# MarvinLvn/CPC2

Measured on AMD Instinct MI355X. Metric: audio-seconds/sec CPC training (1.28 s @16 kHz, 128 neg), higher is better.
Workload: dtype f32

## Files before the change

cpc2_amd/_lib.py:

```python
import ctypes
import os
import time

import torch

_HERE = os.path.dirname(os.path.abspath(__file__))
LIB_PATH = os.environ.get("CPC2_HIP_LIB") or os.path.join(_HERE, "libcpc2_hip.so")

c_float_p = ctypes.c_void_p
c_ptr = ctypes.c_void_p
c_int = ctypes.c_int
c_long = ctypes.c_long
c_size_t = ctypes.c_size_t
c_float = ctypes.c_float

SIGNATURES = {
    "cpc_version": (c_int, []),
    "cpc_last_error": (ctypes.c_char_p, []),
    "cpc_async_error_check": (c_int, [c_ptr]),
    "cpc_prof_enable": (c_int, [c_int]),
    "cpc_gemm_set_mode": (c_int, [c_int]),
    "cpc_prof_read": (c_int, [ctypes.c_char_p, ctypes.POINTER(ctypes.c_double), ctypes.POINTER(c_long)]),
    "cpc_gemm_nt": (c_int, [c_ptr, c_long, c_ptr, c_long, c_ptr, c_long, c_ptr, c_int, c_int, c_int, c_ptr]),
    "cpc_gemm_tn_scratch_bytes": (c_size_t, [c_int, c_int, c_long]),
# ... 42 lines not shown
    "cpc_negidx_sample_host": (c_int, [c_ptr, c_int, c_int, c_int, c_int, c_int, c_ptr, c_ptr, c_ptr]),
    "cpc_negidx_sample_host_async": (c_int, [c_ptr, c_int, c_int, c_int, c_int, c_int, c_ptr]),
    "cpc_negidx_wait": (c_int, [c_ptr]),
    "cpc_mt_draw_host": (c_int, [c_ptr, c_ptr, c_size_t]),
    "cpc_mt_draw_host_async": (c_int, [c_ptr, c_ptr, c_size_t]),
    "cpc_mt_draw_device_async": (c_int, [c_ptr, c_ptr, c_ptr, c_size_t, c_int, c_ptr]),
    "cpc_mt_draw_expand_device_async": (c_int, [c_ptr, c_ptr, c_ptr, c_ptr, c_int, c_int, c_int, c_int, c_int, c_ptr]),
    "cpc_mt_redraw_expand_device_async": (c_int, [c_ptr, c_ptr, c_int, c_int, c_size_t, c_ptr, c_ptr, c_ptr, c_int, c_int, c_int, c_int, c_int, c_ptr]),
    "cpc_negidx_wait_on": (c_int, [c_ptr, c_ptr]),
    "cpc_negidx_stream": (c_int, [c_ptr, c_ptr]),
    "cpc_stream_create_apart": (c_int, [c_ptr, c_int, c_ptr]),
    "cpc_streams_overlap": (c_int, [c_ptr, c_ptr]),
    "cpc_stream_apart_failures": (c_long, []),
    "cpc_stream_spin": (c_int, [c_ptr, c_long]),
    "cpc_side_stream": (c_int, [c_ptr, c_ptr]),
    "cpc_negidx_expand": (c_int, [c_ptr, c_ptr, c_int, c_int, c_int, c_int, c_ptr]),
    "cpc_infonce_saved_bytes": (c_size_t, [c_int] * 6),
    "cpc_infonce_scratch_bytes": (c_size_t, [c_int] * 6),
    "cpc_infonce_logits_offset": (c_size_t, [c_int] * 6),
    "cpc_infonce_perm_offset": (c_size_t, [c_int] * 6),
    "cpc_infonce_forward": (c_int, [c_ptr] * 9 + [c_int] * 7 + [c_ptr]),
    "cpc_infonce_backward": (c_int, [c_ptr] * 11 + [c_int] * 8 + [c_ptr]),
    "cpc_infonce_join": (c_int, [c_ptr]),
    "cpc_infonce_forward_pred": (c_int, [c_ptr] * 8 + [c_int] * 5 + [c_ptr]),
    "cpc_infonce_backward_pred": (c_int, [c_ptr] * 9 + [c_int] * 5 + [c_ptr]),
    "cpc_flac_info": (c_int, [ctypes.c_char_p, ctypes.POINTER(c_int), ctypes.POINTER(c_int), ctypes.POINTER(c_int),
                              ctypes.POINTER(c_long)]),
    "cpc_flac_decode_f32": (c_int, [ctypes.c_char_p, c_ptr, c_long, ctypes.POINTER(c_int)]),
    "cpc_window_gather": (c_int, [c_ptr, c_long, c_ptr, c_ptr, c_int, c_int, c_ptr]),
    "cpc_adam_step": (c_int, [c_ptr, c_ptr, c_ptr, c_ptr, c_long, c_int, c_float, c_float, c_float, c_float, c_float, c_ptr]),
    "cpc_sgd_step": (c_int, [c_ptr, c_ptr, c_ptr, c_long, c_int, c_float, c_float, c_float, c_ptr]),
    "cpc_abx_dtw_scratch_bytes": (c_size_t, [c_int, c_int, c_int]),
    "cpc_abx_dtw": (c_int, [c_ptr, c_int, c_ptr, c_ptr, c_int, c_ptr, c_ptr, c_ptr, c_int, c_int, c_int, c_int, c_ptr, c_ptr,
                            c_ptr, c_size_t, c_ptr]),
    "cpc_abx_counts": (c_int, [c_ptr, c_int, c_ptr, c_ptr, c_ptr, c_int, c_ptr, c_ptr, c_ptr]),
    "cpc_abx_dtw_units_scratch_bytes": (c_size_t, [c_int, c_int, c_int]),
    "cpc_abx_dtw_units": (c_int, [c_ptr, c_ptr, c_ptr, c_int, c_ptr, c_ptr, c_ptr, c_int, c_int, c_int, c_float, c_float, c_ptr,
                                  c_ptr, c_ptr, c_size_t, c_ptr]),
    "cpc_kmeans_scratch_bytes": (c_size_t, [c_long, c_int, c_int]),
    "cpc_kmeans_assign": (c_int, [c_ptr, c_long, c_int, c_ptr, c_int, c_ptr, c_ptr, c_ptr]),
    "cpc_kmeans_distances": (c_int, [c_ptr, c_long, c_int, c_ptr, c_int, c_ptr, c_ptr]),
    "cpc_kmeans_accumulate": (c_int, [c_ptr, c_long, c_int, c_ptr, c_int, c_ptr, c_ptr, c_ptr, c_size_t, c_ptr]),
    "cpc_probe_xent": (c_int, [c_ptr, c_ptr, c_long, c_int, c_int, c_ptr, c_ptr, c_ptr, c_ptr, c_ptr]),
    "cpc_probe_xent_backward_scratch_bytes": (c_size_t, [c_int]),
    "cpc_probe_head_backward": (c_int, [c_ptr, c_long, c_int, c_ptr, c_ptr, c_ptr, c_size_t, c_ptr]),
    "cpc_probe_ctc_scratch_bytes": (c_size_t, [c_int, c_int, c_int]),
# ... 117 lines not shown
```

cpc2_amd/csrc/infonce.hip:

```cpp
#include "common.h"
#include <hip/hip_ext.h>
#include "coop.h"
#include "ldsdma.h"
#include "rowcfg.h"

#include <algorithm>
#include <atomic>
#include <cstdlib>
#include <map>
#include <mutex>

namespace cpc {

typedef float f32x4 __attribute__((ext_vector_type(4)));
typedef float f32x16 __attribute__((ext_vector_type(16)));

constexpr int NCE_ROWS = 16;
constexpr int NCE_POS = 16;

struct NceArgs {
    const float *Pk[16];
    float *dPk[16];
    long p_stride;
    int p_rows;
    int p_packed;
    const float *z;
    const int32_t *ext;
    const unsigned short *perm;
    const float *weights;
    float *logits;
    float *lse;
    float *lossp;
    float *hit;
    int b, T, W, K, Nneg;
    int lw;
    const float *dloss;
    float *vbuf;
    float *ds_buf;
    float inv_count;
};

__global__ __launch_bounds__(64) void nce_block_sort_kernel(const int32_t *ext, int32_t *sorted, unsigned short *perm, int Nneg,
                                                            int rows_per_block, int nblk, int nrows, int *err)
{
    const long base = (long)blockIdx.x * Nneg;
    const int lane = threadIdx.x;
    int pos = 0;
    bool bad = false;
    for (int blk = 0; blk < nblk; ++blk)
        for (int c = 0; c < Nneg; c += 64) {
            const int j = c + lane;
            int row = j < Nneg ? ext[base + j] : -1;
            if (j < Nneg && (unsigned)row >= (unsigned)nrows) { bad = true; row = 0; }
            const bool mine = j < Nneg && min(row / rows_per_block, nblk - 1) == blk;
            const unsigned long long m = __ballot(mine);
            if (mine) {
                const int at = pos + __popcll(m & ((1ull << lane) - 1ull));
                sorted[base + at] = row;
                perm[base + at] = (unsigned short)j;
            }
            pos += __popcll(m);
// ... 467 lines not shown
#pragma unroll
        for (int kp = 0; kp < NCE_ROWS / 2; ++kp) av[kp] = dS[(2 * kp + h) * a.lw + ct * 32 + r32];
        int voff[16];
#pragma unroll
        for (int e = 0; e < 16; ++e) {
            const int ci = ct * 32 + (e & 3) + 8 * (e >> 2) + 4 * h;
            voff[e] = rowidx[ci] >= 0 ? (ci < NCE_POS ? ci : ci - NCE_POS + a.K) * H : -1;
        }
#pragma unroll
        for (int dt = 0; dt < DT32; ++dt) {
            f32x16 acc;
#pragma unroll
            for (int e = 0; e < 16; ++e) acc[e] = 0.f;
#pragma unroll
            for (int kp = 0; kp < NCE_ROWS / 2; ++kp) acc = __builtin_amdgcn_mfma_f32_32x32x2f32(av[kp], bvals[dt][kp], acc, 0, 0, 0);
#pragma unroll
            for (int e = 0; e < 16; ++e)
                if (voff[e] >= 0) vb[voff[e] + dt * 32] = acc[e];
        }
    }
}

constexpr int NCE_SROW = 68;
template <int H, int NKK> __global__ __launch_bounds__(H / 2) void infonce_bwd_fused_kernel(NceArgs a)
{
    constexpr int NW = H / 128;
    extern __shared__ __attribute__((aligned(16))) float smem[];
    float *dS = smem;
    int *rowidx = reinterpret_cast<int *>(dS + NCE_ROWS * a.lw);
    float *stage0 = reinterpret_cast<float *>(rowidx + a.lw);
    const int wave = threadIdx.x >> 6, lane = threadIdx.x & 63, r = lane & 15, q = lane >> 4;
    float *stage = stage0 + wave * 16 * NCE_SROW;

    const int bb = blockIdx.x / a.p_rows, t = blockIdx.x - bb * a.p_rows;
    if (t >= a.W) {
        for (int k = 0; k < a.K; ++k) {
            float *row = a.dPk[k] + ((long)bb * a.p_rows + t) * a.p_stride;
            for (int i = threadIdx.x; i < H / 4; i += 64 * NW) reinterpret_cast<float4 *>(row)[i] = make_float4(0.f, 0.f, 0.f, 0.f);
        }
        return;
    }
    const long bt = (long)bb * a.W + t;
    const int ncand = NCE_POS + a.Nneg;
    const int npad = a.lw - 4;
    const float inv_h = 1.f / H;
    const float wgt = (a.weights != nullptr ? a.weights[bt] : 1.f) * a.inv_count;

// ... 25 lines not shown
            const int neg = a.ext[bt * a.Nneg + j];
            const int pos = (g < a.K && t + 1 + g < a.T) ? bb * a.T + t + 1 + g : -1;
            rowidx[g] = g < NCE_POS ? pos : (g < ncand ? neg : -1);
        }
#pragma unroll
        for (int i = 0; i < NT; ++i)
            if ((int)threadIdx.x + 64 * NW * i < n) stage0[threadIdx.x + 64 * NW * i] = tmp[i];
    }
    __syncthreads();
#pragma unroll
    for (int kk = 0; kk < KW; ++kk) {
        const int k = wave + NW * kk, kc = min(k, a.K - 1);
#pragma unroll
        for (int i = 0; i < GI; ++i) {
            const int g = lane + 64 * i;
            const float e = expf(stage0[kc * lrow + gi[i]] - lsek[kk]);
            float v = g >= NCE_POS ? (g < ncand ? coef[kk] * e : 0.f) : (g == k ? coef[kk] * (e - 1.f) : 0.f);
            if (k >= a.K) v = 0.f;
            if (g < a.lw) dS[k * a.lw + g] = v;
        }
    }
    __syncthreads();

    const int d0 = 128 * wave;
    const long prow_off = ((long)bb * a.p_rows + t) * a.p_stride + d0;
    float pa[8][NKK];
#pragma unroll
    for (int kk = 0; kk < NKK; ++kk) {
        const int k = 4 * kk + q;
        const float *pk = a.Pk[min(k, a.K - 1)] + prow_off + r;
#pragma unroll
        for (int tile = 0; tile < 8; ++tile) {
            const float v = pk[16 * tile];
            pa[tile][kk] = k < a.K ? v : 0.f;
        }
    }
    float *vb = a.vbuf + (bt * (long)ncand + q) * H + d0 + 4 * r;
#define NCE_ROWS_GROUP(C0)                                                                                                     \
    {                                                                                                                          \
        const int c0_ = (C0);                                                                                                  \
        float bv[NKK];                                                                                                         \
        _Pragma("unroll") for (int kk = 0; kk < NKK; ++kk) bv[kk] = dS[(4 * kk + q) * a.lw + c0_ + r];                        \
        _Pragma("unroll") for (int half = 0; half < 2; ++half) {                                                               \
            f32x4 acc[4];                                                                                                      \
            _Pragma("unroll") for (int tl = 0; tl < 4; ++tl) acc[tl] = (f32x4){0.f, 0.f, 0.f, 0.f};                            \
            _Pragma("unroll") for (int kk = 0; kk < NKK; ++kk)                                                                 \
                _Pragma("unroll") for (int tl = 0; tl < 4; ++tl)                                                               \
                    acc[tl] = __builtin_amdgcn_mfma_f32_16x16x4f32(pa[4 * half + tl][kk], bv[kk], acc[tl], 0, 0, 0);           \
            _Pragma("unroll") for (int tl = 0; tl < 4; ++tl)                                                                   \
                *reinterpret_cast<f32x4 *>(stage + r * NCE_SROW + 16 * tl + 4 * q) = acc[tl];                                  \
            __builtin_amdgcn_fence(__ATOMIC_RELEASE, "wavefront");                                                             \
            __builtin_amdgcn_wave_barrier();                                                                                   \
            float4 v[4];                                                                                                       \
            _Pragma("unroll") for (int j = 0; j < 4; ++j)                                                                      \
                v[j] = *reinterpret_cast<const float4 *>(stage + (4 * j + q) * NCE_SROW + 4 * r);                              \
            _Pragma("unroll") for (int j = 0; j < 4; ++j)                                                                      \
                __builtin_nontemporal_store(__builtin_bit_cast(f32x4, v[j]),                                                   \
// ... 16 lines not shown
                const int g = 4 * (s0 + u) + q;
                const int row = rowidx[g];
                bv4[buf][u] = dS[r * a.lw + g];
                const float *src = a.z + (long)(row >= 0 ? row : 0) * H + d0 + 4 * r;
                av[buf][u][0] = *reinterpret_cast<const float4 *>(src);
                av[buf][u][1] = *reinterpret_cast<const float4 *>(src + 64);
            }
        };
        auto multiply = [&](int buf) {
#pragma unroll
            for (int u = 0; u < 4; ++u)
#pragma unroll
                for (int T4 = 0; T4 < 2; ++T4) {
                    dp[T4][0] = __builtin_amdgcn_mfma_f32_16x16x4f32(av[buf][u][T4].x, bv4[buf][u], dp[T4][0], 0, 0, 0);
                    dp[T4][1] = __builtin_amdgcn_mfma_f32_16x16x4f32(av[buf][u][T4].y, bv4[buf][u], dp[T4][1], 0, 0, 0);
                    dp[T4][2] = __builtin_amdgcn_mfma_f32_16x16x4f32(av[buf][u][T4].z, bv4[buf][u], dp[T4][2], 0, 0, 0);
                    dp[T4][3] = __builtin_amdgcn_mfma_f32_16x16x4f32(av[buf][u][T4].w, bv4[buf][u], dp[T4][3], 0, 0, 0);
                }
        };
        const int nb = npad / 16;
        request(0, 0);
        for (int ib = 0; ib < nb; ib += 2) {
            request(1, 4 * (ib + 1));
            NCE_ROWS_GROUP(16 * ib)
            multiply(0);
            if (ib + 2 < nb) request(0, 4 * (ib + 2));
            if (16 * (ib + 1) < ncand) NCE_ROWS_GROUP(16 * (ib + 1))
            multiply(1);
        }
        if (r < a.K) {
            float *dprow = a.dPk[r] + ((long)bb * a.p_rows + t) * a.p_stride + d0;
#pragma unroll
            for (int T4 = 0; T4 < 2; ++T4)
#pragma unroll
                for (int reg = 0; reg < 4; ++reg)
                    *reinterpret_cast<float4 *>(dprow + 64 * T4 + 16 * q + 4 * reg) =
                        make_float4(dp[T4][0][reg], dp[T4][1][reg], dp[T4][2][reg], dp[T4][3][reg]);
        }
    }
#undef NCE_ROWS_GROUP
}

__global__ void nce_hist_kernel(const int32_t *ext, long n, int *counts)
{
    for (long o = (long)blockIdx.x * blockDim.x + threadIdx.x; o < n; o += (long)gridDim.x * blockDim.x)
        atomicAdd(counts + ext[o], 1);
}

__global__ __launch_bounds__(1024) void nce_scan_kernel(const int *counts, int rows, int *offsets)
{
// ... 85 lines not shown
        for (int i = 0; i < 8; ++i)
#pragma unroll
            for (int c = 0; c < PER; ++c)
                v[i][c] = lane + 64 * c < C4 ? nt_load4(v4 + (long)src[i] * C4 + lane + 64 * c) : make_float4(0.f, 0.f, 0.f, 0.f);
#pragma unroll
        for (int i = 0; i < 8; ++i)
#pragma unroll
            for (int c = 0; c < PER; ++c) { acc[c].x += v[i][c].x; acc[c].y += v[i][c].y; acc[c].z += v[i][c].z; acc[c].w += v[i][c].w; }
    }
    for (; e > beg; --e) {
        const int o = entries[e - 1];
        add_row((long)(o / Nneg) * vrows + pos_rows + o % Nneg);
    }
    for (int k = 0; k < K; ++k) {
        const int t = tp - 1 - k;
        if (t >= 0 && t < W) add_row(((long)bb * W + t) * vrows + k);
    }
#pragma unroll
    for (int c = 0; c < PER; ++c)
        if (lane + 64 * c < C4) reinterpret_cast<float4 *>(dz)[(long)r * C4 + lane + 64 * c] = acc[c];
    }
}

__global__ void negidx_expand_kernel(const uint32_t *raw, int32_t *ext, int b, int T, int W, int Nneg)
{
    const long n = (long)b * Nneg * W;
    for (long o = (long)blockIdx.x * blockDim.x + threadIdx.x; o < n; o += (long)gridDim.x * blockDim.x) {
        const int nn = (int)(o % Nneg);
        const long bt = o / Nneg;
        const int t = (int)(bt % W), bb = (int)(bt / W);
        const long i = ((long)bb * Nneg + nn) * W + t;
        const uint32_t bi = raw[i] % (uint32_t)b;
        uint32_t seq = raw[n + i] % (uint32_t)(T - 1) + 1u + (uint32_t)t;
        if (seq >= (uint32_t)T) seq -= (uint32_t)T;
        ext[o] = (int32_t)(seq + bi * (uint32_t)T);
    }
}

struct NceLayout {
    int b, T, K, W, Har, Henc, Nneg, lw;
    int Pr;
    float *P, *logits, *lse;
    int32_t *ext_sorted;
    unsigned short *perm;
    int nblk, rows_per_block;
    size_t saved_bytes;
    float *lossp, *hit, *dP, *wt, *tn, *tn_late;
    float *vbuf;
    float *ds_buf;
    int *counts, *offsets, *entries;
    size_t tn_bytes, scratch_bytes;
    size_t lds_fwd, lds_bwd, lds_bwd_fused;
};

static bool nce_supported(int H) { return H == 32 || H == 64 || H == 128 || H == 256 || H == 512; }

static int nce_layout(NceLayout &l, int b, int T, int K, int Har, int Henc, int Nneg, void *saved, void *scratch)
{
    CPC_REQUIRE(nce_supported(Henc), "infonce: encoder dim %d not supported (32, 64, 128, 256, 512)", Henc);
    CPC_REQUIRE(b > 0 && K >= 1 && K <= 16 && T > K && Nneg >= 1 && Har >= 1,
                "infonce: bad shape b=%d T=%d K=%d (1..16) dim_ar=%d n_neg=%d", b, T, K, Har, Nneg);
    l.b = b; l.T = T; l.K = K; l.W = T - K; l.Har = Har; l.Henc = Henc; l.Nneg = Nneg; l.Pr = T;
    l.lw = (int)cdiv(NCE_POS + Nneg, 32) * 32 + 4;
    Carver sv(saved);
    l.P = sv.take<float>((size_t)b * T * K * Henc);
    l.logits = sv.take<float>((size_t)b * l.W * K * (Nneg + 1));
    l.lse = sv.take<float>((size_t)b * l.W * K);
    l.ext_sorted = sv.take<int32_t>((size_t)b * l.W * Nneg);
    l.perm = sv.take<unsigned short>((size_t)b * l.W * Nneg + 1024);
    const size_t zbytes = sizeof(float) * (size_t)b * T * Henc;
    l.nblk = (int)std::min<size_t>(16, std::max<size_t>(1, (zbytes + (1u << 21) - 1) >> 21));
    l.rows_per_block = (int)cdiv((long)b * T, l.nblk);
    l.saved_bytes = sv.used();
    Carver sc(scratch);
    l.lossp = sc.take<float>((size_t)b * l.W * K);
    l.hit = sc.take<float>((size_t)b * l.W * K);
    l.dP = sc.take<float>((size_t)b * T * K * Henc);
    l.wt = sc.take<float>((size_t)K * Henc * Har);
    l.tn_bytes = std::max(gemm_tn_scratch_bytes(K * Henc, Har, (long)b * T), gemm_nt_scratch_bytes((long)b * T, Har, K * Henc));
    l.tn = sc.take<float>(l.tn_bytes / sizeof(float));
    l.tn_late = sc.take<float>(l.tn_bytes / sizeof(float));
    l.counts = sc.take<int>((size_t)b * T);
    l.offsets = sc.take<int>((size_t)b * T + 1);
    l.entries = sc.take<int>((size_t)b * l.W * Nneg);
    l.vbuf = sc.take<float>((size_t)b * l.W * (NCE_POS + Nneg) * Henc);
    l.ds_buf = sc.take<float>((size_t)b * l.W * (NCE_ROWS + 1) * l.lw);
    l.scratch_bytes = sc.used();
    l.lds_fwd = align_up(sizeof(int) * (size_t)Nneg + sizeof(unsigned short) * (size_t)Nneg, 16);
    l.lds_bwd = sizeof(float) * (size_t)NCE_ROWS * l.lw + sizeof(int) * (size_t)l.lw;
    CPC_REQUIRE(l.lds_bwd <= 64 * 1024, "infonce: n_neg=%d needs %zu B of LDS (> 64 KiB)", Nneg, l.lds_bwd);
    l.lds_bwd_fused = l.lds_bwd + sizeof(float) * (size_t)(Henc / 128) * 16 * NCE_SROW;
    return CPC_OK;
}

template <typename Kern> static int allow_lds(Kern kern, size_t bytes)
{
    if (bytes > 64 * 1024)
        CPC_CHECK_HIP(hipFuncSetAttribute(reinterpret_cast<const void *>(kern), hipFuncAttributeMaxDynamicSharedMemorySize, (int)bytes));
    return CPC_OK;
}

#define NCE_DISPATCH(H, ...)                                    \
    switch (H) {                                                \
    case 32: { constexpr int HH = 32; __VA_ARGS__; } break;    \
    case 64: { constexpr int HH = 64; __VA_ARGS__; } break;    \
    case 128: { constexpr int HH = 128; __VA_ARGS__; } break;  \
    case 256: { constexpr int HH = 256; __VA_ARGS__; } break;  \
    case 512: { constexpr int HH = 512; __VA_ARGS__; } break;  \
    default: break;                                             \
// ... 41 lines not shown
                if (status == CPC_OK && e0 != nullptr) hipExtLaunchKernelGGL(infonce_fwd_dma_kernel<512>, dim3(grid), dim3(64), lds, st, e0, e1, 0, a, n_bt);
                else if (status == CPC_OK) hipLaunchKernelGGL(infonce_fwd_dma_kernel<512>, dim3(grid), dim3(64), lds, st, a, n_bt);
            }
        } else {
            NCE_DISPATCH(l.Henc, {
                status = allow_lds(infonce_fwd_kernel<HH>, l.lds_fwd);
                if (status == CPC_OK) hipLaunchKernelGGL(infonce_fwd_kernel<HH>, dim3((unsigned)(l.b * l.W)), dim3(64), l.lds_fwd, st, a);
            });
        }
        if (status != CPC_OK) prof.cancel();
    }
    CPC_TRY(status);
    CPC_CHECK_LAUNCH("infonce_fwd_kernel");
    hipLaunchKernelGGL(infonce_reduce_kernel, dim3(2 * l.K), dim3(256), 0, st, l.lossp, l.hit, (long)l.b * l.W, l.K, a.inv_count, losses, acc);
    CPC_CHECK_LAUNCH("infonce_reduce_kernel");
    return CPC_OK;
}

struct NceSide {
    hipStream_t stream = nullptr;
    hipEvent_t fork = nullptr, join = nullptr;
    hipEvent_t mid = nullptr, late = nullptr;
    std::atomic<bool> pending{false};
    bool marked = false, started = false, late_fused = false;
    NceLayout l;
    float *dz = nullptr, *dwpred = nullptr;
    const float *c = nullptr;
};

static int nce_side(NceSide **out, hipStream_t caller)
{
    static std::mutex mu;
    static std::map<int, NceSide> sides;
    int dev = 0;
    CPC_CHECK_HIP(hipGetDevice(&dev));
    std::lock_guard<std::mutex> lk(mu);
    NceSide &sd = sides[dev];
    if (sd.stream == nullptr) {
        CPC_TRY(side_stream_get(caller, &sd.stream));
        CPC_CHECK_HIP(hipEventCreateWithFlags(&sd.fork, hipEventDisableTiming));
        CPC_CHECK_HIP(hipEventCreateWithFlags(&sd.join, hipEventDisableTiming));
        CPC_CHECK_HIP(hipEventCreateWithFlags(&sd.mid, hipEventDisableTiming));
        CPC_CHECK_HIP(hipEventCreateWithFlags(&sd.late, hipEventDisableTiming));
    }
    *out = &sd;
    return CPC_OK;
}

static int nce_launch_gather(const NceLayout &l, float *dz, bool fused, hipStream_t st)
{
    const int rows = l.b * l.T;
    const unsigned wgs = (unsigned)cdiv(rows, 4);
    NCE_DISPATCH(l.Henc, hipLaunchKernelGGL(infonce_dz_gather_kernel<HH>, dim3(wgs), dim3(256), 0, st, l.vbuf,
                                             l.offsets, l.entries, dz, l.b, l.T, l.W, l.K, l.Nneg, fused ? NCE_POS : l.K));
    CPC_CHECK_LAUNCH("infonce_dz_gather_kernel");
    return CPC_OK;
}

static int nce_launch_bwd(NceArgs &a, const NceLayout &l, float *dz, hipStream_t st, NceSide **late = nullptr)
{
    const long n = (long)l.b * l.W * l.Nneg;
    const int rows = l.b * l.T;
    a.vbuf = l.vbuf;
    a.ds_buf = l.ds_buf;
    ProfScope prof(PROF_NCE_BWD, st);
    NceSide *side = nullptr;
    CPC_TRY(nce_side(&side, st));
    CPC_CHECK_HIP(hipEventRecord(side->fork, st));
    CPC_CHECK_HIP(hipStreamWaitEvent(side->stream, side->fork, 0));
    const unsigned blocks = (unsigned)std::min<long>(cdiv(n, 256), 4096);
    CPC_CHECK_HIP(hipMemsetAsync(l.counts, 0, sizeof(int) * (size_t)rows, side->stream));
    hipLaunchKernelGGL(nce_hist_kernel, dim3(blocks), dim3(256), 0, side->stream, a.ext, n, l.counts);
    hipLaunchKernelGGL(nce_scan_kernel, dim3(1), dim3(1024), 0, side->stream, l.counts, rows, l.offsets);
    CPC_CHECK_HIP(hipMemsetAsync(l.counts, 0, sizeof(int) * (size_t)rows, side->stream));
    hipLaunchKernelGGL(nce_fill_kernel, dim3(blocks), dim3(256), 0, side->stream, a.ext, n, l.offsets, l.counts, l.entries);
    hipLaunchKernelGGL(nce_sort_kernel, dim3((unsigned)cdiv(rows, 4)), dim3(256), 0, side->stream, l.offsets, l.entries, rows);
    CPC_CHECK_LAUNCH("infonce reference lists");
    CPC_CHECK_HIP(hipEventRecord(side->join, side->stream));
    int status = CPC_OK;
    const bool fused = (l.Henc == 256 || l.Henc == 512) && a.perm != nullptr && l.lw <= 320 &&
                       l.Nneg % 16 == 0 && (size_t)l.K * (l.Nneg + 1) <= (size_t)(l.Henc / 128) * 16 * NCE_SROW;
    if (fused) {
        const unsigned grid = (unsigned)(l.b * a.p_rows);
#define NCE_FUSED(HH, NKK)                                                                                                  \
    {                                                                                                                       \
        status = allow_lds(infonce_bwd_fused_kernel<HH, NKK>, l.lds_bwd_fused);                                             \
        if (status == CPC_OK) hipLaunchKernelGGL((infonce_bwd_fused_kernel<HH, NKK>), dim3(grid), dim3(HH / 2), l.lds_bwd_fused, st, a); \
    }
        const int nkk = (l.K + 3) / 4;
        if (l.Henc == 256) {
            if (nkk == 1) NCE_FUSED(256, 1) else if (nkk == 2) NCE_FUSED(256, 2) else if (nkk == 3) NCE_FUSED(256, 3) else NCE_FUSED(256, 4)
        } else {
            if (nkk == 1) NCE_FUSED(512, 1) else if (nkk == 2) NCE_FUSED(512, 2) else if (nkk == 3) NCE_FUSED(512, 3) else NCE_FUSED(512, 4)
        }
#undef NCE_FUSED
    } else {
        NCE_DISPATCH(l.Henc, {
            status = allow_lds(infonce_bwd_kernel<HH>, l.lds_bwd);
            if (status == CPC_OK) hipLaunchKernelGGL(infonce_bwd_kernel<HH>, dim3((unsigned)(l.b * a.p_rows)), dim3(64), l.lds_bwd, st, a);
        });
    }
    CPC_TRY(status);
    CPC_CHECK_LAUNCH("infonce_bwd_kernel");
    if (!fused) {
        NCE_DISPATCH(l.Henc, hipLaunchKernelGGL(infonce_dz_store_kernel<HH>, dim3((unsigned)(l.b * l.W)), dim3(64), l.lds_bwd, st, a));
        CPC_CHECK_LAUNCH("infonce_dz_store_kernel");
    }
    if (late != nullptr) {
        *late = side;
        side->late_fused = fused;
        return CPC_OK;
    }
    CPC_CHECK_HIP(hipStreamWaitEvent(st, side->join, 0));
    CPC_TRY(nce_launch_gather(l, dz, fused, st));
    return CPC_OK;
}

static int infonce_forward(const float *c, const float *z, const float *wpred, const int32_t *ext, const float *weights,
                           float *losses, float *acc, void *saved, void *scratch, int b, int T, int K, int Har, int Henc,
                           int Nneg, int c_frames, hipStream_t st)
{
    NceLayout l;
    CPC_TRY(nce_layout(l, b, T, K, Har, Henc, Nneg, saved, scratch));
    CPC_REQUIRE(c_frames == T || c_frames == l.W, "infonce: the context holds %d frames per window (expected %d or %d)", c_frames, T, l.W);
    l.Pr = c_frames;
    RowMap none{};
    CPC_TRY(gemm_nt(c, Har, wpred, Har, l.P, (long)K * Henc, nullptr, (long)b * l.Pr, K * Henc, Har, none, st));
    CPC_TRY(nce_sort_negatives(l, ext, st));
    NceArgs a{};
    nce_common(a, l, z, ext, weights);
    for (int k = 0; k < K; ++k) a.Pk[k] = l.P + (size_t)k * Henc;
    a.p_stride = (long)K * Henc; a.p_rows = l.Pr;
    a.p_packed = (size_t)b * T * K * Henc * sizeof(float) < (1ull << 32) ? 1 : 0;
    return nce_launch_fwd(a, l, losses, acc, st);
}

static int infonce_backward(const float *c, const float *z, const float *wpred, const int32_t *ext, const float *weights,
                            const float *dlosses, void *saved, void *scratch, float *dc, float *dz, float *dwpred, int b, int T,
                            int K, int Har, int Henc, int Nneg, int c_frames, bool defer, hipStream_t st)
{
    NceLayout l;
    CPC_TRY(nce_layout(l, b, T, K, Har, Henc, Nneg, saved, scratch));
    CPC_REQUIRE(c_frames == T || c_frames == l.W, "infonce: the context holds %d frames per window (expected %d or %d)", c_frames, T, l.W);
    l.Pr = c_frames;
    NceArgs a{};
    nce_common(a, l, z, ext, weights);
    for (int k = 0; k < K; ++k) { a.Pk[k] = l.P + (size_t)k * Henc; a.dPk[k] = l.dP + (size_t)k * Henc; }
    a.p_stride = (long)K * Henc; a.p_rows = l.Pr;
    a.dloss = dlosses;
    NceSide *late = nullptr;
    CPC_TRY(nce_launch_bwd(a, l, dz, st, defer ? &late : nullptr));
    CPC_TRY(transpose2d(wpred, l.wt, K * Henc, Har, st));
    RowMap none{};
    none.splitk_scratch = l.tn; none.splitk_bytes = l.tn_bytes;
    CPC_TRY(gemm_nt(l.dP, (long)K * Henc, l.wt, (long)K * Henc, dc, Har, nullptr, (long)b * l.Pr, Har, K * Henc, none, st));
    if (late != nullptr) {
        late->l = l; late->dz = dz; late->dwpred = dwpred; late->c = c;
        late->started = false; late->marked = false;
        late->pending.store(true);
    } else {
        CPC_TRY(gemm_tn(l.dP, (long)K * Henc, c, Har, dwpred, Har, K * Henc, Har, (long)b * l.Pr, l.tn, l.tn_bytes, 0, 0, st));
    }
    return CPC_OK;
}

int infonce_deferred_mark(hipStream_t st)
{
    NceSide *side = nullptr;
    CPC_TRY(nce_side(&side, st));
    if (!side->pending.load() || side->started || side->marked) return CPC_OK;
    CPC_CHECK_HIP(hipEventRecord(side->mid, st));
    side->marked = true;
    return CPC_OK;
}

int infonce_deferred_start(hipStream_t st)
{
    NceSide *side = nullptr;
    CPC_TRY(nce_side(&side, st));
    if (!side->pending.load() || side->started) return CPC_OK;
    const NceLayout &l = side->l;
    CPC_TRY(infonce_deferred_mark(st));
    CPC_CHECK_HIP(hipStreamWaitEvent(side->stream, side->mid, 0));
    CPC_TRY(nce_launch_gather(l, side->dz, side->late_fused, side->stream));
    CPC_TRY(gemm_tn(l.dP, (long)l.K * l.Henc, side->c, l.Har, side->dwpred, l.Har, l.K * l.Henc, l.Har, (long)l.b * l.Pr, l.tn_late, l.tn_bytes, 0,
                    0, side->stream));
    CPC_CHECK_HIP(hipEventRecord(side->late, side->stream));
    side->started = true;
    return CPC_OK;
}

static int infonce_join(hipStream_t st)
{
    NceSide *side = nullptr;
    CPC_TRY(nce_side(&side, st));
    if (side->pending.load()) {
        CPC_TRY(infonce_deferred_start(st));
        {
            ProfScope held(PROF_SIDE_WAIT, st);
            CPC_CHECK_HIP(hipStreamWaitEvent(st, side->late, 0));
        }
        side->pending.store(false);
    }
    return CPC_OK;
}

static int infonce_forward_pred(const float *const *pred, const float *z, const int32_t *ext, const float *weights, float *losses,
                                float *acc, void *saved, void *scratch, int b, int T, int K, int Henc, int Nneg, hipStream_t st)
{
    NceLayout l;
    CPC_TRY(nce_layout(l, b, T, K, Henc, Henc, Nneg, saved, scratch));
    CPC_TRY(nce_sort_negatives(l, ext, st));
    NceArgs a{};
    nce_common(a, l, z, ext, weights);
    for (int k = 0; k < K; ++k) a.Pk[k] = pred[k];
    a.p_stride = Henc; a.p_rows = l.W;
    return nce_launch_fwd(a, l, losses, acc, st);
}

static int infonce_backward_pred(const float *const *pred, const float *z, const int32_t *ext, const float *weights,
                                 const float *dlosses, void *saved, void *scratch, float *const *dpred, float *dz, int b, int T, int K,
                                 int Henc, int Nneg, hipStream_t st)
{
    NceLayout l;
    CPC_TRY(nce_layout(l, b, T, K, Henc, Henc, Nneg, saved, scratch));
    NceArgs a{};
    nce_common(a, l, z, ext, weights);
    for (int k = 0; k < K; ++k) { a.Pk[k] = pred[k]; a.dPk[k] = dpred[k]; }
    a.p_stride = Henc; a.p_rows = l.W;
    a.dloss = dlosses;
    return nce_launch_bwd(a, l, dz, st);
}

}

extern "C" int cpc_negidx_expand(const uint32_t *raw, int32_t *ext_idx, int batch, int seq_len, int window, int n_neg,
                                 cpc_stream_t stream)
{
    CPC_REQUIRE(raw != nullptr && ext_idx != nullptr && batch >= 1 && seq_len >= 2 && window >= 1 && window <= seq_len && n_neg >= 1 &&
                    (long long)batch * seq_len <= 2147483647LL,
                "cpc_negidx_expand: bad arguments (batch=%d seq_len=%d window=%d n_neg=%d)", batch, seq_len, window, n_neg);
    const long n = (long)batch * n_neg * window;
    hipLaunchKernelGGL(cpc::negidx_expand_kernel, dim3((unsigned)std::min<long>(cpc::cdiv(n, 256), 2048)), dim3(256), 0,
                       static_cast<hipStream_t>(stream), raw, ext_idx, batch, seq_len, window, n_neg);
    CPC_CHECK_LAUNCH("negidx_expand_kernel");
    return CPC_OK;
}

extern "C" size_t cpc_infonce_saved_bytes(int b, int t, int k, int dim_ar, int dim_enc, int n_neg)
{
    cpc::NceLayout l;
    if (cpc::nce_layout(l, b, t, k, dim_ar, dim_enc, n_neg, nullptr, nullptr) != CPC_OK) return 0;
    return l.saved_bytes;
}

extern "C" size_t cpc_infonce_logits_offset(int b, int t, int k, int dim_ar, int dim_enc, int n_neg)
{
    cpc::NceLayout l;
    char *const base = reinterpret_cast<char *>(4096);
    if (cpc::nce_layout(l, b, t, k, dim_ar, dim_enc, n_neg, base, nullptr) != CPC_OK) return (size_t)-1;
    return (size_t)(reinterpret_cast<char *>(l.logits) - base);
}

extern "C" size_t cpc_infonce_perm_offset(int b, int t, int k, int dim_ar, int dim_enc, int n_neg)
{
    cpc::NceLayout l;
    char *const base = reinterpret_cast<char *>(4096);
    if (cpc::nce_layout(l, b, t, k, dim_ar, dim_enc, n_neg, base, nullptr) != CPC_OK) return (size_t)-1;
    return (size_t)(reinterpret_cast<char *>(l.perm) - base);
}

extern "C" size_t cpc_infonce_scratch_bytes(int b, int t, int k, int dim_ar, int dim_enc, int n_neg)
{
    cpc::NceLayout l;
    if (cpc::nce_layout(l, b, t, k, dim_ar, dim_enc, n_neg, nullptr, nullptr) != CPC_OK) return 0;
    return l.scratch_bytes;
}

extern "C" int cpc_infonce_forward(const float *c, const float *z, const float *wpred, const int32_t *ext_idx, const float *weights,
                                   float *losses, float *acc, void *saved, void *scratch, int b, int t, int c_frames, int k, int dim_ar,
                                   int dim_enc, int n_neg, cpc_stream_t stream)
{
    return cpc::infonce_forward(c, z, wpred, ext_idx, weights, losses, acc, saved, scratch, b, t, k, dim_ar, dim_enc, n_neg, c_frames,
                                static_cast<hipStream_t>(stream));
}

extern "C" int cpc_infonce_backward(const float *c, const float *z, const float *wpred, const int32_t *ext_idx, const float *weights,
                                    const float *dlosses, void *saved, void *scratch, float *dc, float *dz, float *dwpred, int b,
                                    int t, int c_frames, int k, int dim_ar, int dim_enc, int n_neg, int deferred, cpc_stream_t stream)
{
    return cpc::infonce_backward(c, z, wpred, ext_idx, weights, dlosses, saved, scratch, dc, dz, dwpred, b, t, k, dim_ar, dim_enc,
                                 n_neg, c_frames, deferred != 0, static_cast<hipStream_t>(stream));
}

// ... 18 lines not shown
```

include/cpc2_hip.h:

```cpp
#ifndef CPC2_HIP_H
#define CPC2_HIP_H

#include <stddef.h>
#include <stdint.h>

#ifdef __cplusplus
extern "C" {
#endif

typedef void *cpc_stream_t;

enum cpc_status {
    CPC_OK = 0,
    CPC_ERR_INVALID = -1,
    CPC_ERR_HIP = -2,
    CPC_ERR_WORKSPACE = -3
};

int cpc_version(void);
const char *cpc_last_error(void);

int cpc_async_error_check(cpc_stream_t stream);

int cpc_stream_create_apart(const cpc_stream_t *avoid, int n_avoid, cpc_stream_t *out);
// ... 100 lines not shown
                             cpc_stream_t caller_stream);
int cpc_mt_draw_expand_device_async(cpc_mt19937 *g, uint32_t *raw_host, uint32_t *raw_dev, int32_t *ext_dev, int device,
                                    int batch, int seq_len, int window, int n_neg, cpc_stream_t caller_stream);
int cpc_mt_redraw_expand_device_async(cpc_mt19937 *g, const uint32_t *restore_mt624, int restore_left, int restore_next,
                                      size_t skip_words, uint32_t *raw_host, uint32_t *raw_dev, int32_t *ext_dev, int device,
                                      int batch, int seq_len, int window, int n_neg, cpc_stream_t caller_stream);
int cpc_negidx_wait_on(cpc_mt19937 *g, cpc_stream_t stream);
int cpc_negidx_stream(cpc_mt19937 *g, cpc_stream_t *out);
int cpc_negidx_expand(const uint32_t *raw, int32_t *ext_idx, int batch, int seq_len, int window, int n_neg,
                      cpc_stream_t stream);

size_t cpc_infonce_saved_bytes(int b, int t, int k, int dim_ar, int dim_enc, int n_neg);
size_t cpc_infonce_scratch_bytes(int b, int t, int k, int dim_ar, int dim_enc, int n_neg);
size_t cpc_infonce_logits_offset(int b, int t, int k, int dim_ar, int dim_enc, int n_neg);
size_t cpc_infonce_perm_offset(int b, int t, int k, int dim_ar, int dim_enc, int n_neg);
int cpc_infonce_forward(const float *c, const float *z, const float *wpred, const int32_t *ext_idx,
                        const float *weights, float *losses, float *acc, void *saved, void *scratch,
                        int b, int t, int c_frames, int k, int dim_ar, int dim_enc, int n_neg, cpc_stream_t stream);
int cpc_infonce_backward(const float *c, const float *z, const float *wpred, const int32_t *ext_idx,
                         const float *weights, const float *dlosses, void *saved, void *scratch,
                         float *dc, float *dz, float *dwpred, int b, int t, int c_frames, int k, int dim_ar,
                         int dim_enc, int n_neg, int deferred, cpc_stream_t stream);
int cpc_infonce_join(cpc_stream_t stream);

int cpc_infonce_forward_pred(const float *const *pred, const float *z, const int32_t *ext_idx, const float *weights,
                             float *losses, float *acc, void *saved, void *scratch, int b, int t, int k,
                             int dim_enc, int n_neg, cpc_stream_t stream);
int cpc_infonce_backward_pred(const float *const *pred, const float *z, const int32_t *ext_idx,
                              const float *weights, const float *dlosses, void *saved, void *scratch,
                              float *const *dpred, float *dz, int b, int t, int k, int dim_enc, int n_neg,
                              cpc_stream_t stream);

int cpc_flac_info(const char *path, int *sample_rate, int *channels, int *bits_per_sample,
                  long *total_samples);
int cpc_flac_decode_f32(const char *path, float *out_host, long capacity_floats, int *md5_ok);

int cpc_window_gather(const float *audio, long total_samples, const long *offsets, float *out, int batch,
                      int window, cpc_stream_t stream);

int cpc_adam_step(float *p, const float *g, float *m, float *v, long n, int step, float lr,
                  float beta1, float beta2, float eps, float grad_scale, cpc_stream_t stream);

int cpc_sgd_step(float *p, const float *g, float *buf, long n, int step, float lr, float momentum,
                 float grad_scale, cpc_stream_t stream);

enum cpc_abx_distance { CPC_ABX_COSINE = 0, CPC_ABX_EUCLIDIAN = 1 };
// ... 56 lines not shown
```

Baseline: 17640.

## Compute InfoNCE dz via context-space product then single GEMM with prediction weights

For the linear predictor case, the backward no longer forms per-candidate prediction rows to accumulate dz. It writes transposed score gradients, accumulates U = sum of dS times context vectors in the smaller AR dimension with MFMA, and then computes dz as U times a reordered copy of the prediction weights in one GEMM. This reassociation avoids loading the K prediction rows in the fused kernel and the gather of them, at the cost of extra scratch (ds_t, U, wcat), a weight-reorder kernel each step, and an additional GEMM.

```diff
diff --git a/cpc2_amd/_lib.py b/cpc2_amd/_lib.py
--- a/cpc2_amd/_lib.py
+++ b/cpc2_amd/_lib.py
@@ -88,6 +88,7 @@
     "cpc_infonce_forward": (c_int, [c_ptr] * 9 + [c_int] * 7 + [c_ptr]),
     "cpc_infonce_backward": (c_int, [c_ptr] * 11 + [c_int] * 8 + [c_ptr]),
     "cpc_infonce_join": (c_int, [c_ptr]),
+    "cpc_infonce_dz_form": (c_int, [c_int] * 6),
     "cpc_infonce_forward_pred": (c_int, [c_ptr] * 8 + [c_int] * 5 + [c_ptr]),
     "cpc_infonce_backward_pred": (c_int, [c_ptr] * 9 + [c_int] * 5 + [c_ptr]),
     "cpc_flac_info": (c_int, [ctypes.c_char_p, ctypes.POINTER(c_int), ctypes.POINTER(c_int), ctypes.POINTER(c_int),
diff --git a/cpc2_amd/csrc/infonce.hip b/cpc2_amd/csrc/infonce.hip
--- a/cpc2_amd/csrc/infonce.hip
+++ b/cpc2_amd/csrc/infonce.hip
@@ -37,6 +37,7 @@
     const float *dloss;
     float *vbuf;
     float *ds_buf;
+    float *ds_t;
     float inv_count;
 };
 
@@ -550,7 +551,7 @@
 }
 
 constexpr int NCE_SROW = 68;
-template <int H, int NKK> __global__ __launch_bounds__(H / 2) void infonce_bwd_fused_kernel(NceArgs a)
+template <int H, int NKK, bool ROWS> __global__ __launch_bounds__(H / 2) void infonce_bwd_fused_kernel(NceArgs a)
 {
     constexpr int NW = H / 128;
     extern __shared__ __attribute__((aligned(16))) float smem[];
@@ -622,17 +623,27 @@
     }
     __syncthreads();
 
+    if constexpr (!ROWS) {
+        float4 *out = reinterpret_cast<float4 *>(a.ds_t) + bt * (long)ncand * 4;
+        for (int i = threadIdx.x; i < ncand * 4; i += 64 * NW) {
+            const int g = i >> 2, k4 = 4 * (i & 3);
+            out[i] = make_float4(dS[k4 * a.lw + g], dS[(k4 + 1) * a.lw + g], dS[(k4 + 2) * a.lw + g], dS[(k4 + 3) * a.lw + g]);
+        }
+    }
+
     const int d0 = 128 * wave;
     const long prow_off = ((long)bb * a.p_rows + t) * a.p_stride + d0;
     float pa[8][NKK];
-#pragma unroll
-    for (int kk = 0; kk < NKK; ++kk) {
-        const int k = 4 * kk + q;
-        const float *pk = a.Pk[min(k, a.K - 1)] + prow_off + r;
-#pragma unroll
-        for (int tile = 0; tile < 8; ++tile) {
-            const float v = pk[16 * tile];
-            pa[tile][kk] = k < a.K ? v : 0.f;
+    if constexpr (ROWS) {
+#pragma unroll
+        for (int kk = 0; kk < NKK; ++kk) {
+            const int k = 4 * kk + q;
+            const float *pk = a.Pk[min(k, a.K - 1)] + prow_off + r;
+#pragma unroll
+            for (int tile = 0; tile < 8; ++tile) {
+                const float v = pk[16 * tile];
+                pa[tile][kk] = k < a.K ? v : 0.f;
+            }
         }
     }
     float *vb = a.vbuf + (bt * (long)ncand + q) * H + d0 + 4 * r;
@@ -695,10 +706,12 @@
         request(0, 0);
         for (int ib = 0; ib < nb; ib += 2) {
             request(1, 4 * (ib + 1));
-            NCE_ROWS_GROUP(16 * ib)
+            if constexpr (ROWS) NCE_ROWS_GROUP(16 * ib)
             multiply(0);
             if (ib + 2 < nb) request(0, 4 * (ib + 2));
-            if (16 * (ib + 1) < ncand) NCE_ROWS_GROUP(16 * (ib + 1))
+            if constexpr (ROWS) {
+                if (16 * (ib + 1) < ncand) NCE_ROWS_GROUP(16 * (ib + 1))
+            }
             multiply(1);
         }
         if (r < a.K) {
@@ -830,6 +843,93 @@
     }
 }
 
+constexpr int NCE_U_CHUNK = 256;
+template <int HAR> __global__ __launch_bounds__(HAR / 2, 8) void infonce_dz_ctx_kernel(const float *c, const float *ds_t,
+                                                                                      const int *offsets, const int *entries,
+                                                                                      float *U, int T, int W, int K, int Nneg, int Pr)
+{
+    __shared__ int2 refs[NCE_U_CHUNK];
+    const int row = blockIdx.x;
+    const int bb = row / T, tp = row - bb * T;
+    const int wave = threadIdx.x >> 6, lane = threadIdx.x & 63, r = lane & 15, q = lane >> 4;
+    const int d0 = 128 * wave;
+    const int ncand = NCE_POS + Nneg;
+    const int beg = offsets[row], n = offsets[row + 1] - beg;
+    const int total = n + K;
+
+    f32x4 acc[2][4];
+#pragma unroll
+    for (int T4 = 0; T4 < 2; ++T4)
+#pragma unroll
+        for (int e = 0; e < 4; ++e) acc[T4][e] = (f32x4){0.f, 0.f, 0.f, 0.f};
+
+    for (int base = 0; base < total; base += NCE_U_CHUNK) {
+        const int cnt = min(NCE_U_CHUNK, total - base), cnt8 = (cnt + 7) & ~7;
+        if (base > 0) __syncthreads();
+        for (int i = threadIdx.x; i < cnt8; i += HAR / 2) {
+            const int idx = base + i;
+            int crow = 0, gran = -1;
+            if (idx < n) {
+                const unsigned o = (unsigned)entries[beg + idx];
+                const unsigned bt = o / (unsigned)Nneg, slot = o - bt * (unsigned)Nneg;
+                const unsigned b2 = bt / (unsigned)W, t2 = bt - b2 * (unsigned)W;
+                crow = (int)(b2 * (unsigned)Pr + t2);
+                gran = (int)(bt * (unsigned)ncand + NCE_POS + slot);
+            } else if (idx < total) {
+                const int k = idx - n, t2 = tp - 1 - k;
+                if (t2 >= 0 && t2 < W) {
+                    crow = bb * Pr + t2;
+                    gran = (bb * W + t2) * ncand + k;
+                }
+            }
+            refs[i] = make_int2(crow, gran);
+        }
+        __syncthreads();
+        for (int s = 0; s < cnt8; s += 8) {
+            float4 av[2][2];
+            float bv[2];
+#pragma unroll
+            for (int u = 0; u < 2; ++u) {
+                const int2 ref = refs[s + 4 * u + q];
+                const float *src = c + (long)ref.x * HAR + d0 + 4 * r;
+                av[u][0] = *reinterpret_cast<const float4 *>(src);
+                av[u][1] = *reinterpret_cast<const float4 *>(src + 64);
+                const float g = ds_t[(long)max(ref.y, 0) * NCE_ROWS + r];
+                bv[u] = ref.y >= 0 ? g : 0.f;
+            }
+#pragma unroll
+            for (int u = 0; u < 2; ++u)
+#pragma unroll
+                for (int T4 = 0; T4 < 2; ++T4) {
+                    acc[T4][0] = __builtin_amdgcn_mfma_f32_16x16x4f32(av[u][T4].x, bv[u], acc[T4][0], 0, 0, 0);
+                    acc[T4][1] = __builtin_amdgcn_mfma_f32_16x16x4f32(av[u][T4].y, bv[u], acc[T4][1], 0, 0, 0);
+                    acc[T4][2] = __builtin_amdgcn_mfma_f32_16x16x4f32(av[u][T4].z, bv[u], acc[T4][2], 0, 0, 0);
+                    acc[T4][3] = __builtin_amdgcn_mfma_f32_16x16x4f32(av[u][T4].w, bv[u], acc[T4][3], 0, 0, 0);
+                }
+        }
+    }
+    if (r < K) {
+        float *urow = U + ((long)row * K + r) * HAR + d0;
+#pragma unroll
+        for (int T4 = 0; T4 < 2; ++T4)
+#pragma unroll
+            for (int reg = 0; reg < 4; ++reg)
+                *reinterpret_cast<float4 *>(urow + 64 * T4 + 16 * q + 4 * reg) =
+                    make_float4(acc[T4][0][reg], acc[T4][1][reg], acc[T4][2][reg], acc[T4][3][reg]);
+    }
+}
+
+__global__ void nce_wcat_kernel(const float4 *wpred, float4 *wcat, int K, int Henc, int Har4)
+{
+    const long n = (long)K * Henc * Har4;
+    for (long o = (long)blockIdx.x * blockDim.x + threadIdx.x; o < n; o += (long)gridDim.x * blockDim.x) {
+        const int a = (int)(o % Har4);
+        const long ke = o / Har4;
+        const int e = (int)(ke % Henc), k = (int)(ke / Henc);
+        wcat[((long)e * K + k) * Har4 + a] = wpred[o];
+    }
+}
+
 __global__ void negidx_expand_kernel(const uint32_t *raw, int32_t *ext, int b, int T, int W, int Nneg)
 {
     const long n = (long)b * Nneg * W;
@@ -857,6 +957,7 @@
     float *vbuf;
     float *ds_buf;
     int *counts, *offsets, *entries;
+    float *ds_t, *U, *wcat;
     size_t tn_bytes, scratch_bytes;
     size_t lds_fwd, lds_bwd, lds_bwd_fused;
 };
@@ -885,7 +986,8 @@
     l.hit = sc.take<float>((size_t)b * l.W * K);
     l.dP = sc.take<float>((size_t)b * T * K * Henc);
     l.wt = sc.take<float>((size_t)K * Henc * Har);
-    l.tn_bytes = std::max(gemm_tn_scratch_bytes(K * Henc, Har, (long)b * T), gemm_nt_scratch_bytes((long)b * T, Har, K * Henc));
+    l.tn_bytes = std::max({gemm_tn_scratch_bytes(K * Henc, Har, (long)b * T), gemm_nt_scratch_bytes((long)b * T, Har, K * Henc),
+                           gemm_nt_scratch_bytes((long)b * T, Henc, K * Har)});
     l.tn = sc.take<float>(l.tn_bytes / sizeof(float));
     l.tn_late = sc.take<float>(l.tn_bytes / sizeof(float));
     l.counts = sc.take<int>((size_t)b * T);
@@ -893,6 +995,9 @@
     l.entries = sc.take<int>((size_t)b * l.W * Nneg);
     l.vbuf = sc.take<float>((size_t)b * l.W * (NCE_POS + Nneg) * Henc);
     l.ds_buf = sc.take<float>((size_t)b * l.W * (NCE_ROWS + 1) * l.lw);
+    l.ds_t = sc.take<float>((size_t)b * l.W * (NCE_POS + Nneg) * NCE_ROWS);
+    l.U = sc.take<float>((size_t)b * T * K * Har);
+    l.wcat = sc.take<float>((size_t)K * Henc * Har);
     l.scratch_bytes = sc.used();
     l.lds_fwd = align_up(sizeof(int) * (size_t)Nneg + sizeof(unsigned short) * (size_t)Nneg, 16);
     l.lds_bwd = sizeof(float) * (size_t)NCE_ROWS * l.lw + sizeof(int) * (size_t)l.lw;
@@ -980,10 +1085,11 @@
     hipEvent_t fork = nullptr, join = nullptr;
     hipEvent_t mid = nullptr, late = nullptr;
     std::atomic<bool> pending{false};
-    bool marked = false, started = false, late_fused = false;
+    bool marked = false, started = false;
+    int late_form = 0;
     NceLayout l;
     float *dz = nullptr, *dwpred = nullptr;
-    const float *c = nullptr;
+    const float *c = nullptr, *wpred = nullptr;
 };
 
 static int nce_side(NceSide **out, hipStream_t caller)
@@ -1005,6 +1111,22 @@
     return CPC_OK;
 }
 
+enum { NCE_DZ_ROWS = 0, NCE_DZ_ROWS_FUSED = 1, NCE_DZ_PRODUCT = 2 };
+static bool nce_fused_ok(const NceLayout &l)
+{
+    return (l.Henc == 256 || l.Henc == 512) && l.lw <= 320 && l.Nneg % 16 == 0 &&
+           (size_t)l.K * (l.Nneg + 1) <= (size_t)(l.Henc / 128) * 16 * NCE_SROW;
+}
+static int nce_dz_form(const NceLayout &l, bool linear)
+{
+    if (!nce_fused_ok(l)) return NCE_DZ_ROWS;
+    return linear && (l.Har == 256 || l.Har == 512) ? NCE_DZ_PRODUCT : NCE_DZ_ROWS_FUSED;
+}
+
+struct NceLinear {
+    const float *c, *wpred;
+};
+
 static int nce_launch_gather(const NceLayout &l, float *dz, bool fused, hipStream_t st)
 {
     const int rows = l.b * l.T;
@@ -1015,12 +1137,34 @@
     return CPC_OK;
 }
 
-static int nce_launch_bwd(NceArgs &a, const NceLayout &l, float *dz, hipStream_t st, NceSide **late = nullptr)
+static int nce_launch_dz(const NceLayout &l, int form, const NceLinear &lin, float *dz, hipStream_t st)
+{
+    if (form != NCE_DZ_PRODUCT) return nce_launch_gather(l, dz, form == NCE_DZ_ROWS_FUSED, st);
+    const int rows = l.b * l.T;
+    if (l.Har == 256)
+        hipLaunchKernelGGL(infonce_dz_ctx_kernel<256>, dim3((unsigned)rows), dim3(128), 0, st, lin.c, l.ds_t, l.offsets, l.entries, l.U,
+                           l.T, l.W, l.K, l.Nneg, l.Pr);
+    else
+        hipLaunchKernelGGL(infonce_dz_ctx_kernel<512>, dim3((unsigned)rows), dim3(256), 0, st, lin.c, l.ds_t, l.offsets, l.entries, l.U,
+                           l.T, l.W, l.K, l.Nneg, l.Pr);
+    CPC_CHECK_LAUNCH("infonce_dz_ctx_kernel");
+    const long n4 = (long)l.K * l.Henc * (l.Har / 4);
+    hipLaunchKernelGGL(nce_wcat_kernel, dim3((unsigned)std::min<long>(cdiv(n4, 256), 2048)), dim3(256), 0, st,
+                       reinterpret_cast<const float4 *>(lin.wpred), reinterpret_cast<float4 *>(l.wcat), l.K, l.Henc, l.Har / 4);
+    CPC_CHECK_LAUNCH("nce_wcat_kernel");
+    RowMap none{};
+    none.splitk_scratch = l.tn_late; none.splitk_bytes = l.tn_bytes;
+    return gemm_nt(l.U, (long)l.K * l.Har, l.wcat, (long)l.K * l.Har, dz, l.Henc, nullptr, rows, l.Henc, l.K * l.Har, none, st);
+}
+
+static int nce_launch_bwd(NceArgs &a, const NceLayout &l, const NceLinear &lin, float *dz, hipStream_t st, NceSide **late = nullptr)
 {
     const long n = (long)l.b * l.W * l.Nneg;
     const int rows = l.b * l.T;
     a.vbuf = l.vbuf;
     a.ds_buf = l.ds_buf;
+    a.ds_t = l.ds_t;
+    const int form = nce_dz_form(l, lin.c != nullptr);
     ProfScope prof(PROF_NCE_BWD, st);
     NceSide *side = nullptr;
     CPC_TRY(nce_side(&side, st));
@@ -1036,22 +1180,26 @@
     CPC_CHECK_LAUNCH("infonce reference lists");
     CPC_CHECK_HIP(hipEventRecord(side->join, side->stream));
     int status = CPC_OK;
-    const bool fused = (l.Henc == 256 || l.Henc == 512) && a.perm != nullptr && l.lw <= 320 &&
-                       l.Nneg % 16 == 0 && (size_t)l.K * (l.Nneg + 1) <= (size_t)(l.Henc / 128) * 16 * NCE_SROW;
+    const bool fused = form != NCE_DZ_ROWS;
     if (fused) {
         const unsigned grid = (unsigned)(l.b * a.p_rows);
-#define NCE_FUSED(HH, NKK)                                                                                                  \
+#define NCE_FUSED_AS(HH, NKK, ROWS)                                                                                         \
     {                                                                                                                       \
-        status = allow_lds(infonce_bwd_fused_kernel<HH, NKK>, l.lds_bwd_fused);                                             \
-        if (status == CPC_OK) hipLaunchKernelGGL((infonce_bwd_fused_kernel<HH, NKK>), dim3(grid), dim3(HH / 2), l.lds_bwd_fused, st, a); \
-    }
+        status = allow_lds(infonce_bwd_fused_kernel<HH, NKK, ROWS>, l.lds_bwd_fused);                                       \
+        if (status == CPC_OK)                                                                                               \
+            hipLaunchKernelGGL((infonce_bwd_fused_kernel<HH, NKK, ROWS>), dim3(grid), dim3(HH / 2), l.lds_bwd_fused, st, a); \
+    }
+#define NCE_FUSED(HH, NKK) NCE_FUSED_AS(HH, NKK, true)
         const int nkk = (l.K + 3) / 4;
-        if (l.Henc == 256) {
+        if (form == NCE_DZ_PRODUCT) {
+            if (l.Henc == 256) NCE_FUSED_AS(256, 1, false) else NCE_FUSED_AS(512, 1, false)
+        } else if (l.Henc == 256) {
             if (nkk == 1) NCE_FUSED(256, 1) else if (nkk == 2) NCE_FUSED(256, 2) else if (nkk == 3) NCE_FUSED(256, 3) else NCE_FUSED(256, 4)
         } else {
             if (nkk == 1) NCE_FUSED(512, 1) else if (nkk == 2) NCE_FUSED(512, 2) else if (nkk == 3) NCE_FUSED(512, 3) else NCE_FUSED(512, 4)
         }
 #undef NCE_FUSED
+#undef NCE_FUSED_AS
     } else {
         NCE_DISPATCH(l.Henc, {
             status = allow_lds(infonce_bwd_kernel<HH>, l.lds_bwd);
@@ -1066,11 +1214,11 @@
     }
     if (late != nullptr) {
         *late = side;
-        side->late_fused = fused;
+        side->late_form = form;
         return CPC_OK;
     }
     CPC_CHECK_HIP(hipStreamWaitEvent(st, side->join, 0));
-    CPC_TRY(nce_launch_gather(l, dz, fused, st));
+    CPC_TRY(nce_launch_dz(l, form, lin, dz, st));
     return CPC_OK;
 }
 
@@ -1107,13 +1255,13 @@
     a.p_stride = (long)K * Henc; a.p_rows = l.Pr;
     a.dloss = dlosses;
     NceSide *late = nullptr;
-    CPC_TRY(nce_launch_bwd(a, l, dz, st, defer ? &late : nullptr));
+    CPC_TRY(nce_launch_bwd(a, l, NceLinear{c, wpred}, dz, st, defer ? &late : nullptr));
     CPC_TRY(transpose2d(wpred, l.wt, K * Henc, Har, st));
     RowMap none{};
     none.splitk_scratch = l.tn; none.splitk_bytes = l.tn_bytes;
     CPC_TRY(gemm_nt(l.dP, (long)K * Henc, l.wt, (long)K * Henc, dc, Har, nullptr, (long)b * l.Pr, Har, K * Henc, none, st));
     if (late != nullptr) {
-        late->l = l; late->dz = dz; late->dwpred = dwpred; late->c = c;
+        late->l = l; late->dz = dz; late->dwpred = dwpred; late->c = c; late->wpred = wpred;
         late->started = false; late->marked = false;
         late->pending.store(true);
     } else {
@@ -1140,7 +1288,7 @@
     const NceLayout &l = side->l;
     CPC_TRY(infonce_deferred_mark(st));
     CPC_CHECK_HIP(hipStreamWaitEvent(side->stream, side->mid, 0));
-    CPC_TRY(nce_launch_gather(l, side->dz, side->late_fused, side->stream));
+    CPC_TRY(nce_launch_dz(l, side->late_form, NceLinear{side->c, side->wpred}, side->dz, side->stream));
     CPC_TRY(gemm_tn(l.dP, (long)l.K * l.Henc, side->c, l.Har, side->dwpred, l.Har, l.K * l.Henc, l.Har, (long)l.b * l.Pr, l.tn_late, l.tn_bytes, 0,
                     0, side->stream));
     CPC_CHECK_HIP(hipEventRecord(side->late, side->stream));
@@ -1187,7 +1335,7 @@
     for (int k = 0; k < K; ++k) { a.Pk[k] = pred[k]; a.dPk[k] = dpred[k]; }
     a.p_stride = Henc; a.p_rows = l.W;
     a.dloss = dlosses;
-    return nce_launch_bwd(a, l, dz, st);
+    return nce_launch_bwd(a, l, NceLinear{nullptr, nullptr}, dz, st);
 }
 
 }
@@ -1228,6 +1376,13 @@
     return (size_t)(reinterpret_cast<char *>(l.perm) - base);
 }
 
+extern "C" int cpc_infonce_dz_form(int b, int t, int k, int dim_ar, int dim_enc, int n_neg)
+{
+    cpc::NceLayout l;
+    if (cpc::nce_layout(l, b, t, k, dim_ar, dim_enc, n_neg, nullptr, nullptr) != CPC_OK) return 0;
+    return cpc::nce_dz_form(l, true) == cpc::NCE_DZ_PRODUCT ? 1 : 0;
+}
+
 extern "C" size_t cpc_infonce_scratch_bytes(int b, int t, int k, int dim_ar, int dim_enc, int n_neg)
 {
     cpc::NceLayout l;
diff --git a/include/cpc2_hip.h b/include/cpc2_hip.h
--- a/include/cpc2_hip.h
+++ b/include/cpc2_hip.h
@@ -146,6 +146,7 @@
                          float *dc, float *dz, float *dwpred, int b, int t, int c_frames, int k, int dim_ar,
                          int dim_enc, int n_neg, int deferred, cpc_stream_t stream);
 int cpc_infonce_join(cpc_stream_t stream);
+int cpc_infonce_dz_form(int b, int t, int k, int dim_ar, int dim_enc, int n_neg);
 
 int cpc_infonce_forward_pred(const float *const *pred, const float *z, const int32_t *ext_idx, const float *weights,
                              float *losses, float *acc, void *saved, void *scratch, int b, int t, int k,
```

Result: faster. 17880, median of 6 (+1.4%).
